# vankxr/qo-100-tools

Hardware: AMD Instinct MI355X
Metric: complex-IQ MSamples/s through 255-tap FIR (higher is better)
Workload: dtype f32

## Files before the change

include/if_fir_debug.h:

```cpp
#ifndef IF_FIR_DEBUG_H
#define IF_FIR_DEBUG_H

#include "if_fir.h"

#ifdef __cplusplus
extern "C" {
#endif

uint8_t if_fir_time_device(if_fir_ctx_t *pCtx, const void *pDevIn, void *pDevOut, uint64_t ullSamples,
                           uint32_t ulWarmup, uint32_t ulReps, float *pfMsPerCall);
uint32_t if_fir_debug_stamps(if_fir_ctx_t *pCtx, uint64_t *pullOut, uint32_t ulWords);
#define IF_FIR_DEBUG_TABLE_FLOATS 21632u
uint32_t if_fir_debug_fft_tables(const float *pfTaps, uint32_t ulTaps, uint32_t bComplexTaps, uint32_t ulDecimation,
                                 uint32_t ulNcoDelta, float *pfOut, uint32_t ulOutFloats);
uint32_t if_fir_debug_fft_tables_bank(const float *pfTaps, uint32_t ulTaps, uint32_t bComplexTaps, uint32_t ulBank, uint32_t ulParity,
                                      float *pfOut, uint32_t ulOutFloats);
uint32_t if_fir_debug_bank_tail(uint32_t ulDecimation, uint32_t bOwnCentres);
uint8_t if_fir_debug_bank_plan(const uint32_t *pulSlots, uint32_t ulChannels, uint32_t *pulOut);
#define IF_FIR_DEBUG_ODD_TABLE_FLOATS 10496u
uint32_t if_fir_debug_fft_tables_odd(const float *pfTaps, uint32_t ulTaps, uint32_t bComplexTaps, uint32_t ulDecimation,
                                     uint32_t ulNcoDelta, float *pfOut, uint32_t ulOutFloats);
uint8_t if_fir_debug_fft_schedule(uint64_t ullBlocks, uint32_t ulWorkgroups, uint32_t bSingleOk, int64_t *pllOut);
uint8_t if_fir_debug_queue_faults(if_fir_ctx_t *pCtx, uint32_t *pulFaults);
uint32_t if_fir_mc_debug_plan(uint32_t ulWorld, uint32_t ulChannels, uint32_t ulRank, uint64_t ullSamples,
                              uint32_t ulInBytes, uint32_t ulTaps, uint32_t ulDecimation, uint64_t ullConsumed,
                              uint64_t ullChunk, uint64_t *pullOut, uint32_t ulMaxOps);

uint8_t if_fir_debug_interp_config(if_fir_interp_t *pCtx, uint32_t bForceFull, uint32_t ulGridLimit);
uint8_t if_fir_debug_interp_seek(if_fir_interp_t *pCtx, uint64_t ullSamples);
uint32_t if_fir_debug_interp_tables(const float *pfTaps, uint32_t ulTaps, uint32_t bComplexTaps, float *pfOut, uint32_t ulOutFloats);
uint8_t if_fir_debug_interp_plan(uint32_t ulTaps, uint32_t ulInterpolation, uint32_t *pulRows, uint32_t *pulHistLen,
                                 uint32_t *pbFftOk);
uint8_t if_fir_debug_combiner_config(if_fir_combiner_t *pCtx, uint32_t ulGridLimit);
uint8_t if_fir_debug_combiner_seek(if_fir_combiner_t *pCtx, uint64_t ullSamples);
uint32_t if_fir_debug_combiner_tables(const float *pfTaps, uint32_t ulTaps, uint32_t bComplexTaps, double dCentre, uint32_t *pulGrid,
                                      int32_t *plResidual, float *pfOut, uint32_t ulOutFloats);
uint8_t if_fir_debug_resamp_config(if_fir_resamp_t *pCtx, uint32_t ulGridLimit, uint32_t *pulTileOutputs);
// ... 8 lines not shown
```

qo-100-tools_amd/csrc/if_fir_fft_dev.h:

```cpp
#pragma once
namespace if_fir
{

typedef float cf __attribute__((ext_vector_type(2)));
typedef float f2v __attribute__((ext_vector_type(2)));
typedef unsigned u2v __attribute__((ext_vector_type(2)));
typedef float f4v_t __attribute__((ext_vector_type(4)));

__device__ __forceinline__ cf cadd(cf a, cf b) { return a + b; }
__device__ __forceinline__ cf csub(cf a, cf b) { return a - b; }

template <bool CONJ>
__device__ __forceinline__ cf cmul_v(cf a, cf w)
{
    cf t, d;
    asm("v_pk_mul_f32 %0, %1, %2 op_sel_hi:[1,0]" : "=v"(t) : "v"(a), "v"(w));
    if (CONJ)
        asm("v_pk_fma_f32 %0, %1, %2, %3 op_sel:[1,1,0] op_sel_hi:[0,1,1] neg_hi:[0,1,0]" : "=v"(d) : "v"(a), "v"(w), "v"(t));
    else
        asm("v_pk_fma_f32 %0, %1, %2, %3 op_sel:[1,1,0] op_sel_hi:[0,1,1] neg_lo:[0,1,0]" : "=v"(d) : "v"(a), "v"(w), "v"(t));
    return d;
}
template <bool CONJ>
__device__ __forceinline__ cf cmul_s(cf a, cf w)
// ... 493 lines not shown
        const unsigned u = rem + off, qd = __umul24(u, magic) >> 18;
        const bool keep = (__umul24(qd, sub) == u) && in_range;
        return keep ? (qd - (rem ? 1u : 0u)) * 8u : 0xffffffffu;
    }
};

struct DevQueue
{
    char *qcur;
    char *qtail;
    char *qclaim;
    unsigned int *gqueue;
    unsigned int *tqueue;
    unsigned int *faultw;
    int lane;
    __device__ __forceinline__ unsigned long long *tailw() const { return reinterpret_cast<unsigned long long *>(qtail); }
    __device__ __forceinline__ unsigned tail_claim(unsigned simd)
    {
        unsigned c = 0;
        if (lane == 0)
            c = __hip_atomic_fetch_add(reinterpret_cast<unsigned int *>(qclaim) + simd, 1u, __ATOMIC_RELAXED, __HIP_MEMORY_SCOPE_WORKGROUP);
        return __builtin_amdgcn_readfirstlane(c);
    }
    __device__ __forceinline__ unsigned long long tail_add()
    {
        unsigned long long w = 0;
        if (lane == 0)
            w = __hip_atomic_fetch_add(tailw(), 1ull, __ATOMIC_RELAXED, __HIP_MEMORY_SCOPE_WORKGROUP);
        return uniform(w);
    }
// ... 48 lines not shown
    __device__ __forceinline__ unsigned ticket()
    {
        unsigned t = 0;
        if (lane == 0)
            t = atomicAdd(gqueue, 1u);
        return __builtin_amdgcn_readfirstlane(t);
    }
    __device__ __forceinline__ void fault()
    {
        if (lane == 0)
            atomicAdd(faultw, 1u);
    }
    __device__ __forceinline__ void pause() { __builtin_amdgcn_s_sleep(2); }
    __device__ __forceinline__ unsigned wgs() const { return gridDim.x; }
};
inline hipError_t fft_queue_select(const LaunchArgs &a, uint32_t *qsel)
{
    *qsel = 0;
    if (a.queue_base && a.queue_valid && *a.queue_valid)
        *qsel = *a.queue_base & 1u;
    else
    {
        const hipError_t e = hipMemsetAsync(a.queue, 0, 16, a.stream);
        if (e != hipSuccess)
            return e;
    }
    if (a.queue_base && a.queue_valid)
    {
        *a.queue_base = *qsel ^ 1u;
        *a.queue_valid = true;
    }
    return hipSuccess;
}
inline hipError_t fft_queue_launched(const LaunchArgs &a)
{
    const hipError_t le = hipGetLastError();
    if (le != hipSuccess && a.queue_valid)
        *a.queue_valid = false;
    return le;
}

template <bool PF = true>
__device__ __forceinline__ void inverse_tail256(cf (&a)[16], cf (&c)[16], const f2v *twe, const XAddr &xa, int lane)
{
    xst16<XROW>(xa.wx, a);
// ... 88 lines not shown
```

qo-100-tools_amd/csrc/if_fir_fft_kernel.inc:

```
template <int OVL_ROWS, bool DEC4, bool I16, bool NCO, int CHAN, bool DECN, bool ACC>
__global__ __launch_bounds__(512, 2) IF_FIR_LDS_SINGLE_READS void fir_fft_kernel(const f2v *__restrict__ in_, f2v *__restrict__ out,
                                                        const f2v *__restrict__ tables, const f2v *__restrict__ hist,
                                                        int HL, int64_t N, int32_t n0, int64_t M, int64_t nblocks,
                                                        int64_t nblocks_main, unsigned int *queue, unsigned long long *dbg, int32_t diag,
                                                        uint32_t nco_phi0, uint32_t nco_delta, chan_arg_t<CHAN> chan,
                                                        uint32_t qsel, void *__restrict__ hist_out,
                                                        int32_t decn, int32_t decn_n0, int64_t decn_m, int32_t in_shift)
{
    static_assert(!ACC || (tail_single(CHAN) && OVL_ROWS == 32), "accumulating store: single-channel pipelines, 32 overlap rows");
    static_assert(!DECN || (!DEC4 && CHAN == TAIL_FULL_OR_DEC4), "general decimation = the full-rate pipeline with a selecting store");
    static_assert(tail_valid(CHAN) && (CHAN == TAIL_FULL_OR_DEC4 || DEC4), "every named tail but the first is a decimating one");
    static_assert(tail_has_nco(CHAN) || !NCO, "channels at their own centres: no common offset on top; the decimate-by-4 bank takes no NCO either");
    static_assert(OVL_ROWS >= 4 || (!DEC4 && !ACC), "2 overlap rows: full-rate pipeline (D = 1, odd D) only");
    constexpr bool TAN = tail_wants_tan(CHAN, DEC4);
    constexpr bool TANF = !DEC4;
    constexpr int OVL = 64 * OVL_ROWS;
    constexpr int ISZ = I16 ? 4 : 8;
    const char *in = reinterpret_cast<const char *>(in_);
    constexpr int L = FFT_N - OVL;
    constexpr int LOUT = tail_lout(CHAN, DEC4, L);
    constexpr int EARLY_GROUPS = CHAN == TAIL_DEC4_SUB ? FFT_EARLY_GROUPS_SUB : FFT_EARLY_GROUPS;
    constexpr int LAUX = FFT_LOAD_AUX;
    constexpr int EDGE = OVL_ROWS;
    extern __shared__ __attribute__((aligned(16))) char smem[];
// ... 53 lines not shown
        }
        if (threadIdx.x < Q_RING)
            reinterpret_cast<unsigned long long *>(smem + LDS_Q + 16)[threadIdx.x] = queue_ring_init(threadIdx.x, blockIdx.x, gridDim.x);
        if (threadIdx.x < 4)
            reinterpret_cast<unsigned int *>(smem + LDS_QCLAIM)[threadIdx.x] = 0u;
        if (threadIdx.x == 0)
        {
            *reinterpret_cast<unsigned long long *>(smem + LDS_Q) = queue_cur_init(blockIdx.x, gridDim.x, true);
            *reinterpret_cast<unsigned long long *>(smem + LDS_QTAIL) = 0ull;
            if (blockIdx.x == 0)
            {
                queue[qsel ^ 1u] = 0u;
                queue[2u + (qsel ^ 1u)] = 0u;
            }
        }
    }
    __syncthreads();
    DevQueue dq{smem + LDS_Q, smem + LDS_QTAIL, smem + LDS_QCLAIM, queue + qsel, queue + 2 + qsel, queue + 4, lane};
    const unsigned simd = (unsigned)wid & 3u;
    if (wid == 0)
        queue_start(dq);
    if (hist_out && blockIdx.x == 0 && wid == 0)
    {
        const int64_t keep = (int64_t)HL;
        for (int64_t i = lane; i < keep; i += 64)
        {
            const int64_t gi = N - keep + i, hi = keep + gi;
            if constexpr (I16)
            {
                const int *src = reinterpret_cast<const int *>(in_), *hsrc = reinterpret_cast<const int *>(hist);
                reinterpret_cast<int *>(hist_out)[i] = gi >= 0 ? src[gi] : (hi >= 0 ? hsrc[hi] : 0);
            }
            else
// ... 41 lines not shown
        {                                                                                                        \
            dbg[(((blockIdx.x >> 6) * 2 + wid) * 32 + dbg_it) * 8 + (slot)] = __builtin_amdgcn_s_memrealtime();   \
            dbg[4096 + (((blockIdx.x >> 6) * 2 + wid) * 32 + dbg_it) * 8 + (slot)] = __builtin_amdgcn_s_memtime(); \
        }                                                                                                        \
    } while (0)
#else
#define FFT_STAMP(slot) (void)0
#endif
    unsigned long long st_r0 = 0, st_c0 = 0;
    if (dbg)
    {
        st_r0 = __builtin_amdgcn_s_memrealtime();
        st_c0 = __builtin_amdgcn_s_memtime();
    }
    const unsigned voff = (unsigned)lane * 8u;
    while (blk < nblocks)
    {
        FFT_STAMP(0);
        const int64_t s0 = rb(blk) * L - OVL + n0 - in_shift;
        if (!loaded && !(diag & 1))
        {
            if (s0 >= 0)
            {
                const srd_t srd = make_srd(in + s0 * ISZ, (N - s0) * ISZ);
#pragma unroll
                for (int rho = 0; rho < 4; rho++)
#pragma unroll
                    for (int j = 0; j < 16; j++)
                        load_row<I16, LAUX, EDGE>(r, srd, lane, 4 * j + rho);
            }
// ... 64 lines not shown
#pragma unroll
            for (int j = 0; j < 16; j++)
            {
                if (j == 0)
                    r[phys(i, j)] = t[j];
                else
                {
                    r[phys(i, j)] = cmul_v<false>(t[j], w2[j - 1]);
                }
            }
            }
        }
        FFT_STAMP(3);
        exchange2(r, xa);
        FFT_STAMP(4);
        const int64_t blk_next = queue_take(dq, simd, nblocks_main, nblocks);
        const int64_t s0n = rb(blk_next) * L - OVL + n0 - in_shift;
        const bool next_fast = (blk_next < nblocks) && (s0n >= 0) && !(diag & 1);
        const srd_t nsrd = make_srd(in + (next_fast ? s0n : 0) * ISZ, next_fast ? (N - s0n) * ISZ : 0);
        const int64_t obase = rb(blk) * LOUT;
        const srd_t osrd = make_srd(out + obase, (diag & 2) ? 0 : (M - obase) * 8);
        if constexpr (NCO && (CHAN == TAIL_BANK16_ALL || CHAN == TAIL_BANK8_ALL))
        {
            const float2 pb = phasor(nco_phi0 + nco_delta * (uint32_t)obase);
            if (lane == 0)
                *reinterpret_cast<cf *>(smem + LDS_QNCO + wid * 8) = (cf){pb.x, pb.y};
        }
        if constexpr (tail_is_bank(CHAN))
        {
#include "if_fir_fft_tails_bank.inc"
        }
// ... 22 lines not shown
```

qo-100-tools_amd/csrc/if_fir_fft_launch.inc:

```
template <int OVL_ROWS, bool DEC4, bool I16, bool NCO, int CHAN, bool DECN, bool ACC>
static constexpr auto fft_kernel_of()
{
#ifdef IF_FIR_FFT_DEC2_UNIT
    static_assert(tail_in_dec2_units(CHAN), "the decimate-by-2 units hold the decimate-by-2 tails only");
#else
    static_assert(!tail_in_dec2_units(CHAN), "the decimate-by-2 tails live in the decimate-by-2 units (launch_fft_dec2_rows)");
#endif
    return &fir_fft_kernel<OVL_ROWS, DEC4, I16, NCO, CHAN, DECN, ACC>;
}
template <int ROWS>
hipError_t launch_fft_dec2_rows(const LaunchArgs &a, int tail, bool nco, bool acc);
template <int OVL_ROWS, bool DEC4, bool I16, bool NCO, int CHAN, bool DECN, bool ACC>
static hipError_t launch_fft_t(const LaunchArgs &a)
{
    auto kern = fft_kernel_of<OVL_ROWS, DEC4, I16, NCO, CHAN, DECN, ACC>();
    constexpr int L = FFT_N - 64 * OVL_ROWS;
    constexpr int LOUT = tail_lout(CHAN, DEC4, L);
    static DeviceSetup setup;
    int ncus = 0;
    {
        const hipError_t e = device_setup(setup, a.device, reinterpret_cast<const void *>(kern), FFT_LDS_BYTES, &ncus);
        if (e != hipSuccess)
            return e;
    }
    constexpr int F = tail_factor(CHAN, DEC4);
    ChanArgs ca = a.chan ? *a.chan : ChanArgs{};
    ca.sub = tail_sub_word(CHAN, DEC4, a.D, ca.sub);
    const bool both = CHAN == TAIL_BANK8_ALL && (ca.sub & 2u);
    const int64_t m_rate = DECN ? a.N : CHAN == TAIL_BANK8_ALL ? a.M : (a.M - 1) * (int64_t)ca.sub + 1;
    const int32_t n0_rate = DECN ? 0 : a.n0;
    const int64_t nblocks = (a.M > 0 ? (m_rate + LOUT - 1) / LOUT : 0) * (both ? 2 : 1);
    if (nblocks <= 0)
        return hipSuccess;
    const int64_t wgs_max = (a.grid_limit > 0 && a.grid_limit < ncus) ? a.grid_limit : ncus;
    const FftLaunchPlan plan = fft_launch_plan(nblocks, wgs_max, !both && !(a.diag & 262144),
                                               (a.diag & 256) ? 0 : Q_TAIL_MAX_ROUNDS);
    uint32_t qsel = 0;
    {
        const hipError_t e = fft_queue_select(a, &qsel);
        if (e != hipSuccess)
            return e;
    }
    chan_arg_t<CHAN> cak;
    if constexpr (tail_is_bank(CHAN))
        cak = ca;
    else
        cak.sub = ca.sub;
    hipLaunchKernelGGL(kern, dim3((unsigned)plan.wgs), dim3(512), FFT_LDS_BYTES, a.stream,
                       reinterpret_cast<const f2v *>(a.in), reinterpret_cast<f2v *>(a.out),
                       reinterpret_cast<const f2v *>(a.fft_tables), reinterpret_cast<const f2v *>(a.hist_full), a.hist_len, a.N,
                       n0_rate, m_rate, nblocks, plan.nblocks_main, (unsigned int *)a.queue,
                       (unsigned long long *)a.dbg, (int32_t)a.diag | (plan.single ? 131072 : 0),
                       DECN ? 0u - a.nco_word * a.nco_abs0 : nco_phi0(a),
                       DECN ? 0u - a.nco_word : 0u - a.nco_word * (uint32_t)F,
                       cak, qsel, a.hist_out, (int32_t)a.D, (int32_t)a.n0, a.M,
                       (int32_t)a.in_shift);
    return fft_queue_launched(a);
}

enum { NCO_NEVER, NCO_BOTH, NCO_ALWAYS };
template <int ROWS, bool DEC4, int CHAN, bool DECN = false, bool ACC = false, int FORMS = tail_has_nco(CHAN) ? NCO_BOTH : NCO_NEVER>
static hipError_t launch_fft_form(const LaunchArgs &a, bool nco = false)
{
    static_assert(FORMS == NCO_NEVER || tail_has_nco(CHAN), "this tail has no NCO instantiation");
    if constexpr (FORMS == NCO_BOTH)
        switch ((a.in_i16 ? 2 : 0) | (nco ? 1 : 0))
        {
        case 0: return launch_fft_t<ROWS, DEC4, false, false, CHAN, DECN, ACC>(a);
        case 1: return launch_fft_t<ROWS, DEC4, false, true, CHAN, DECN, ACC>(a);
        case 2: return launch_fft_t<ROWS, DEC4, true, false, CHAN, DECN, ACC>(a);
        default: return launch_fft_t<ROWS, DEC4, true, true, CHAN, DECN, ACC>(a);
// ... 8 lines not shown
hipError_t launch_fft_dec2_rows(const LaunchArgs &a, int tail, bool nco, bool acc)
{
    const bool plain = tail == TAIL_DEC2;
    if constexpr (ROWS == 32)
        if (acc)
            return plain ? launch_fft_form<ROWS, true, TAIL_DEC2, false, true>(a, nco) : launch_fft_form<ROWS, true, TAIL_DEC2_SUB, false, true>(a, nco);
    if (acc)
        return hipErrorInvalidConfiguration;
    return plain ? launch_fft_form<ROWS, true, TAIL_DEC2>(a, nco) : launch_fft_form<ROWS, true, TAIL_DEC2_SUB>(a, nco);
}
#if defined(IF_FIR_FFT_ONLY)
__attribute__((used)) static auto *const if_fir_fft_only_kernel = &fir_fft_kernel<IF_FIR_FFT_ONLY>;
#elif defined(IF_FIR_FFT_HAZARD_PROBE)
template __global__ void fir_fft_kernel<IF_FIR_FFT_ROWS, true, false, false, TAIL_DEC2, false, false>(
    const f2v *, f2v *, const f2v *, const f2v *, int, int64_t, int32_t, int64_t, int64_t, int64_t, unsigned int *,
    unsigned long long *, int32_t, uint32_t, uint32_t, chan_arg_t<TAIL_DEC2>, uint32_t, void *, int32_t, int32_t, int64_t, int32_t);
#else
template hipError_t launch_fft_dec2_rows<IF_FIR_FFT_ROWS>(const LaunchArgs &a, int tail, bool nco, bool acc);
#endif
#else
template <int ROWS>
static hipError_t launch_fft_bank8(const LaunchArgs &a, const FftRoute &r)
{
    bool general = a.chan->general || r.sub != 1;
    for (uint32_t c = 0; c < a.chan->count; c++)
        general = general || (a.chan->bin[c] & 255u) || a.chan->pword[c] != (a.chan->bin[c] << 20) + a.nco_word;
    if (general)
        return launch_fft_form<ROWS, true, TAIL_BANK8_CHANNEL, false, false, NCO_ALWAYS>(a);
    const bool nco = a.nco_word != 0;
    const ChanArgs &cin = *a.chan;
    uint32_t pmask[2], rest = 0;
// ... 127 lines not shown
```

qo-100-tools_amd/csrc/if_fir_fft_queue.h:

```cpp
#pragma once
#include <stdint.h>

#if defined(__HIPCC__)
#define IF_FIR_Q_FN __host__ __device__ inline __attribute__((always_inline))
#else
#define IF_FIR_Q_FN inline __attribute__((always_inline))
#endif

namespace if_fir
{

constexpr unsigned QB = 8;
constexpr unsigned Q_AHEAD = 2;
constexpr unsigned Q_RING = 4;
constexpr unsigned Q_SPIN_LIMIT = 1u << 22;
constexpr int64_t Q_NONE = (int64_t)1 << 46;

IF_FIR_Q_FN unsigned long long queue_word(unsigned global_group, unsigned local_group, unsigned slot)
{
    return ((unsigned long long)global_group << 32) | ((unsigned long long)(local_group & 0xffffffu) << 8) | slot;
}
IF_FIR_Q_FN unsigned long long queue_entry(unsigned global_group, unsigned local_group)
{
    return ((unsigned long long)global_group << 32) | local_group;
// ... 93 lines not shown
                break;
            p.pause();
        }
    }
    p.fault();
    return Q_NONE;
}

constexpr int64_t Q_TAIL_MAX_ROUNDS = 6;
IF_FIR_Q_FN int64_t queue_main_blocks(int64_t nblocks, int64_t wgs, int64_t max_rounds = Q_TAIL_MAX_ROUNDS)
{
    const int64_t simds = 4 * wgs, p = nblocks / (2 * simds), rem = nblocks - 2 * p * simds;
    return (p >= 1 && p <= max_rounds && rem > 0 && rem <= simds) ? 2 * p * simds : nblocks;
}

struct FftLaunchPlan
{
    int64_t wgs;
    int64_t nblocks_main;
    int64_t tickets;
    bool single;
};
IF_FIR_Q_FN FftLaunchPlan fft_launch_plan(int64_t nblocks, int64_t wgs_max, bool single_ok, int64_t tail_rounds)
{
    const int64_t groups = (nblocks + QB - 1) / QB;
    FftLaunchPlan p;
    p.single = single_ok && nblocks <= (int64_t)QB * wgs_max;
    const int64_t want = p.single ? nblocks : groups;
    p.wgs = want < wgs_max ? want : wgs_max;
    if (p.wgs < 1)
        p.wgs = 1;
    p.nblocks_main = p.single ? nblocks : queue_main_blocks(nblocks, p.wgs, tail_rounds);
    p.tickets = groups + 2 * p.wgs;
    return p;
}

IF_FIR_Q_FN unsigned long long queue_cur_init(unsigned wg, unsigned wgs, bool static_first)
{
    return static_first ? queue_word(wgs + wg, 1, 0) : queue_word(wg, 0, 0);
}
IF_FIR_Q_FN unsigned long long queue_ring_init(unsigned i, unsigned wg, unsigned wgs)
{
    return i < Q_AHEAD ? queue_entry(i * wgs + wg, i) : ~0ull;
}

}
```

qo-100-tools_amd/csrc/if_fir_kernels.h:

```cpp
#pragma once
#include <hip/hip_runtime.h>
#include <stdint.h>

#include <mutex>

#include "if_fir_fft_route.h"

namespace if_fir
{

enum
{
    BACKEND_AUTO = 0,
    BACKEND_DIRECT = 1,
    BACKEND_TAPSPLIT = 2,
    BACKEND_GENERIC = 3,
    BACKEND_FFT = 4
};

constexpr int CHAN_MAX = 16;
struct ChanArgs
{
    uint32_t count;
    uint32_t slot[CHAN_MAX];
    float tw[CHAN_MAX][30];
    float rot0[CHAN_MAX][2];
    float2 *out[CHAN_MAX];
    uint32_t mask16;
    uint32_t rot_e;
    uint32_t sub;
    uint32_t bin[CHAN_MAX];
    uint32_t pword[CHAN_MAX];
    uint32_t abs0n0;
    uint32_t general;
};

struct LaunchArgs
{
    const void *in;
    void *out;
    const float *taps;
    const void *hist;
    const void *hist_full;
    int hist_len;
    int T, D;
    int in_i16;
    int ctaps;
    int64_t N;
    int32_t n0;
    int64_t M;
    int backend;
    int device;
    hipStream_t stream;
    const void *fft_tables;
    const void *fft_tables_b;
    int in_shift;
    void *queue;
    int diag;
    int grid_limit;
    void *dbg;
    uint32_t nco_word;
    uint32_t nco_abs0;
    void *hist_out;
    uint32_t *queue_base;
    bool *queue_valid;
    int no_fold;
    const ChanArgs *chan;
};

inline uint32_t nco_phi0(const LaunchArgs &a) { return 0u - a.nco_word * (a.nco_abs0 + (uint32_t)a.n0); }
inline uint32_t nco_delta(const LaunchArgs &a) { return 0u - a.nco_word * (uint32_t)a.D; }

#if defined(__HIPCC__)
__device__ __forceinline__ float2 nco_phasor(uint32_t ph)
{
    float sh, ch, sl, cl;
    sincospif((float)(ph >> 16) * (1.0f / 32768.0f), &sh, &ch);
    sincospif((float)(ph & 0xffffu) * (1.0f / 2147483648.0f), &sl, &cl);
    return make_float2(fmaf(ch, cl, -sh * sl), fmaf(sh, cl, ch * sl));
}
// ... 49 lines not shown
```

qo-100-tools_amd/csrc/if_fir_shim.cpp:

```cpp
#include <hip/hip_runtime.h>

#include <cmath>
#include <cstdarg>
#include <cstdio>
#include <cstdlib>
#include <cstring>
#include <new>

#include "if_fir.h"
#ifdef IF_FIR_DEVELOPMENT
#include "if_fir_debug.h"
#endif
#include "if_fir_kernels.h"
#ifdef IF_FIR_DEVELOPMENT
#include "if_fir_fft_queue.h"
#endif

#define IF_FIR_API extern "C" __attribute__((visibility("default")))

struct Tuning
{
    int schedule;
    uint32_t diag;
    int grid_limit;
    bool no_fold;
    bool inject_failure;
    bool needs_debug;
};
static Tuning decode_tuning(uint32_t v)
{
    Tuning t{};
    t.schedule = v <= 6 ? (int)v : 0;
    t.diag = (v >= 1000 && v < 2000) ? v - 1000 : (v >= 1000000 && v < 3000000) ? v - 1000000 : 0;
    t.grid_limit = (v > 2000 && v < 3000) ? (int)(v - 2000) : 0;
    t.no_fold = v == 3000;
    t.inject_failure = v == 4000;
    t.needs_debug = (v >= 1000 && v < 2000) || v == 4000 || v >= 1000000;
    return t;
}

struct if_fir_ctx
{
    int device;
    hipStream_t own_stream;
    hipStream_t stream;
    int T, D;
    int ctaps;
    int in_i16;
    uint32_t backend_req;
    uint32_t backend;
    Tuning tuning;
// ... 5 lines not shown
    uint64_t max_samples;
    void *d_stage_in;
    void *d_stage_out;
    hipStream_t copy_in, copy_out;
    hipEvent_t *chunk_ev;
    uint32_t chunk_ev_count;
    float tone[10];
    float *h_taps;
    uint32_t nco_word;
    float *h_eff;
    void *d_fft_tables;
    void *d_fft_tables_bank;
    void *d_queue;
    uint32_t queue_base;
    bool queue_valid;
    void *d_dbg;
    void *d_power;
    char info[128];
    mutable char err[256];
};

static thread_local char g_init_err[256] = "";

static void set_err(const if_fir_ctx *ctx, const char *fmt, ...)
{
    char *dst = ctx ? ctx->err : g_init_err;
    va_list ap;
    va_start(ap, fmt);
    vsnprintf(dst, 256, fmt, ap);
    va_end(ap);
}
// ... 190 lines not shown
            return 0;                                                                                \
        }                                                                                            \
    } while (0)

    INIT_TRY(hipSetDevice(lDevice));
    hipDeviceProp_t prop;
    INIT_TRY(hipGetDeviceProperties(&prop, lDevice));
    snprintf(ctx->info, sizeof(ctx->info), "%s %s cus=%d clock_mhz=%d lds_per_block=%zu", prop.name, prop.gcnArchName,
             prop.multiProcessorCount, prop.clockRate / 1000, (size_t)prop.sharedMemPerBlock);
    INIT_TRY(hipStreamCreateWithFlags(&ctx->own_stream, hipStreamNonBlocking));
    ctx->stream = ctx->own_stream;
    const size_t taps_padded = ((size_t)tap_floats + 63) / 64 * 64;
    INIT_TRY(hipMalloc((void **)&ctx->d_taps, sizeof(float) * taps_padded));
    INIT_TRY(hipMemset(ctx->d_taps, 0, sizeof(float) * taps_padded));
    INIT_TRY(hipMemcpy(ctx->d_taps, pfTaps, sizeof(float) * tap_floats, hipMemcpyHostToDevice));
    INIT_TRY(hipMalloc(&ctx->d_queue, 32));
    INIT_TRY(hipMemset(ctx->d_queue, 0, 32));
    ctx->hist_len = hist_len_for((int)ulTaps, (int)ulDecimation);
    const size_t hist_bytes = 8 * (size_t)(ctx->hist_len > 0 ? ctx->hist_len : 1);
    for (int i = 0; i < 2; i++)
    {
        INIT_TRY(hipMalloc(&ctx->d_hist[i], hist_bytes));
        INIT_TRY(hipMemset(ctx->d_hist[i], 0, hist_bytes));
    }
#undef INIT_TRY
    ctx->backend_req = IF_FIR_BACKEND_AUTO;
    ctx->backend = resolve_backend(ctx, IF_FIR_BACKEND_AUTO);
    if (ctx->backend == IF_FIR_BACKEND_HIP_FFT && !ensure_fft_tables(ctx))
    {
        snprintf(g_init_err, sizeof(g_init_err), "if_fir_init: %s", ctx->err);
        if_fir_destroy(ctx);
        return 0;
// ... 267 lines not shown
    a.n0 = (int32_t)n0;
    a.M = (int64_t)m;
    a.backend = (int)ctx->backend;
    a.device = ctx->device;
    a.stream = ctx->stream;
    a.fft_tables = ctx->d_fft_tables;
    a.fft_tables_b = (ctx->d_fft_tables && if_fir::fft_two_partitions(ctx->T))
                         ? static_cast<const float *>(ctx->d_fft_tables) + if_fir::FFT_TABLE_FLOATS : nullptr;
    a.queue = ctx->d_queue;
#ifdef IF_FIR_DEVELOPMENT
    a.dbg = ctx->d_dbg;
    const bool fft_var = ctx->backend == IF_FIR_BACKEND_HIP_FFT;
    a.diag = fft_var ? (int)ctx->tuning.diag : 0;
    a.grid_limit = fft_var ? ctx->tuning.grid_limit : 0;
    a.no_fold = ctx->tuning.no_fold;
#endif
    if (chan)
    {
        const bool slots16 = ctx->D == 16 && !chan->general;
        const uint32_t entries = slots16 ? 16u : chan->count;
        for (uint32_t c = 0; c < entries; c++)
        {
            const uint32_t slot = slots16 ? c : chan->slot[c];
            const uint32_t e = (uint32_t)((slot * ((ctx->consumed + n0) & 15u)) & 15u);
            chan->rot0[c][0] = (float)cos(-2.0 * M_PI * (double)e / 16.0);
            chan->rot0[c][1] = (float)sin(-2.0 * M_PI * (double)e / 16.0);
        }
        if (slots16)
        {
            chan->rot_e = (uint32_t)((ctx->consumed + n0) & 15u);
            chan->mask16 = 0;
            for (uint32_t c = 0; c < 16; c++)
                chan->mask16 |= chan->out[c] ? (1u << c) : 0u;
        }
        chan->abs0n0 = (uint32_t)(ctx->consumed + n0);
        a.chan = chan;
        const int kind = if_fir::fft_route_of(a).image.kind;
        if (kind == if_fir::FFT_IMAGE_BANK8 || kind == if_fir::FFT_IMAGE_BANK16)
            a.fft_tables = ctx->d_fft_tables_bank;
        if (kind == if_fir::FFT_IMAGE_BANK8)
            a.fft_tables_b = static_cast<const float *>(ctx->d_fft_tables_bank) + if_fir::FFT_TABLE_FLOATS;
    }
    a.queue_base = &ctx->queue_base;
    a.queue_valid = &ctx->queue_valid;
    const bool fused_history = ctx->backend == IF_FIR_BACKEND_HIP_FFT && m > 0 && ctx->hist_len > 0;
    a.hist_out = fused_history ? ctx->d_hist[ctx->hist_cur ^ 1] : nullptr;
    if (ctx->backend == IF_FIR_BACKEND_HIP_FFT)
        HIP_TRY(ctx, if_fir::launch_fft(a));
    else
        HIP_TRY(ctx, if_fir::launch_fir(a, ctx->tuning.schedule));
    if (!fused_history)
        HIP_TRY(ctx, if_fir::launch_history(in, ctx->d_hist[ctx->hist_cur], ctx->d_hist[ctx->hist_cur ^ 1], ctx->hist_len,
                                            (int64_t)n, ctx->in_i16, ctx->stream));
    if (commit)
    {
        ctx->hist_cur ^= 1;
        ctx->consumed += n;
    }
    return 1;
// ... 305 lines not shown
    HIP_TRY(pCtx, hipStreamSynchronize(pCtx->stream));
    HIP_TRY(pCtx, hipMemcpy(pulFaults, static_cast<const char *>(pCtx->d_queue) + 16, 4, hipMemcpyDeviceToHost));
    return 1;
}

IF_FIR_API uint8_t if_fir_debug_fft_schedule(uint64_t ullBlocks, uint32_t ulWorkgroups, uint32_t bSingleOk, int64_t *pllOut)
{
    if (!pllOut || !ullBlocks || !ulWorkgroups)
        return 0;
    const if_fir::FftLaunchPlan p =
        if_fir::fft_launch_plan((int64_t)ullBlocks, (int64_t)ulWorkgroups, bSingleOk != 0, if_fir::Q_TAIL_MAX_ROUNDS);
    pllOut[0] = p.wgs;
    pllOut[1] = p.nblocks_main;
    pllOut[2] = p.single ? 1 : 0;
    pllOut[3] = p.tickets;
    return 1;
}

#endif

IF_FIR_API uint8_t if_fir_power_device(if_fir_ctx_t *pCtx, const void *pDevIQ, uint64_t ullSamples, double *pdMeanPower)
{
    if (!pCtx || !pdMeanPower)
        return 0;
    *pdMeanPower = 0.0;
    if (ullSamples == 0)
        return 1;
    if (!pDevIQ || ((uintptr_t)pDevIQ & 15))
    {
        set_err(pCtx, "if_fir_power_device: the buffer must be a 16-byte aligned device pointer");
// ... 302 lines not shown
```

qo-100-tools_amd/if_fir.py:

```python
import ctypes
import os

import numpy as np

_HERE = os.path.dirname(os.path.abspath(__file__))
LIB_PATH = os.path.join(_HERE, "libif_fir.so")
DEV_LIB_PATH = os.path.join(_HERE, "libif_fir_dev.so")

INPUT_F32, INPUT_I16 = 0, 1
BACKEND_AUTO, BACKEND_HIP_DIRECT, BACKEND_HIP_TAPSPLIT, BACKEND_HIP_GENERIC, BACKEND_HIP_FFT = range(5)
WINDOW_RECT, WINDOW_HAMMING, WINDOW_HANN, WINDOW_BLACKMAN = range(4)

EXPORTS = [
    "if_bpf_design", "if_bpf_design_complex", "if_fir_init", "if_fir_init_complex", "if_fir_destroy", "if_fir_reset", "if_fir_set_backend", "if_fir_get_backend",
    "if_fir_set_tuning", "if_fir_set_input_format", "if_fir_set_stream", "if_fir_synchronize", "if_fir_last_error", "if_fir_out_count",
    "if_fir_process", "if_fir_process_device", "if_fir_synth_device", "if_fir_dev_alloc",
    "if_fir_dev_free", "if_fir_dev_upload", "if_fir_dev_download", "if_fir_device_info",
    "if_fir_set_nco", "if_fir_get_nco", "if_fir_channelizer_process_device", "if_fir_channelizer_process_device_freq", "if_fir_host_alloc", "if_fir_host_free",
    "if_fir_power_device",
    "if_fir_mc_owner", "if_fir_mc_unique_id", "if_fir_mc_init", "if_fir_mc_destroy", "if_fir_mc_reset",
    "if_fir_mc_set_input_format", "if_fir_mc_process_device", "if_fir_mc_channel_ctx", "if_fir_mc_last_error",
    "if_fir_mc_set_chunk_samples", "if_fir_mc_get_chunk_samples",
    "if_fir_interp_init", "if_fir_interp_init_complex", "if_fir_interp_destroy", "if_fir_interp_reset", "if_fir_interp_set_backend",
    "if_fir_interp_get_backend", "if_fir_interp_set_input_format", "if_fir_interp_set_nco", "if_fir_interp_get_nco",
# ... 2 lines not shown
    "if_fir_resamp_init", "if_fir_resamp_init_complex", "if_fir_resamp_destroy", "if_fir_resamp_reset", "if_fir_resamp_set_input_format",
    "if_fir_resamp_set_stream", "if_fir_resamp_synchronize", "if_fir_resamp_last_error", "if_fir_resamp_out_count",
    "if_fir_resamp_process", "if_fir_resamp_process_device",
    "if_fir_psd_init", "if_fir_psd_destroy", "if_fir_psd_reset", "if_fir_psd_set_input_format", "if_fir_psd_set_stream",
    "if_fir_psd_synchronize", "if_fir_psd_last_error", "if_fir_psd_frame_count", "if_fir_psd_process", "if_fir_psd_process_device",
    "if_fir_combiner_init", "if_fir_combiner_init_complex", "if_fir_combiner_destroy", "if_fir_combiner_reset", "if_fir_combiner_set_backend",
    "if_fir_combiner_get_backend", "if_fir_combiner_set_input_format", "if_fir_combiner_set_centres", "if_fir_combiner_get_centres",
    "if_fir_combiner_set_stream", "if_fir_combiner_synchronize", "if_fir_combiner_last_error", "if_fir_combiner_out_count",
    "if_fir_combiner_process", "if_fir_combiner_process_device",
    "if_fir_ddc_init", "if_fir_ddc_init_complex", "if_fir_ddc_destroy", "if_fir_ddc_reset", "if_fir_ddc_set_input_format",
    "if_fir_ddc_set_nco", "if_fir_ddc_get_nco", "if_fir_ddc_set_stream", "if_fir_ddc_synchronize", "if_fir_ddc_last_error",
    "if_fir_ddc_out_count", "if_fir_ddc_process", "if_fir_ddc_process_device",
]
DEV_EXPORTS = ["if_fir_time_device", "if_fir_debug_stamps", "if_fir_debug_fft_tables", "if_fir_debug_fft_tables_odd", "if_fir_debug_fft_tables_bank",
               "if_fir_debug_bank_plan", "if_fir_debug_bank_tail", "if_fir_debug_fft_schedule",
               "if_fir_mc_debug_plan", "if_fir_debug_queue_faults",
               "if_fir_debug_interp_config", "if_fir_debug_interp_seek", "if_fir_debug_interp_tables", "if_fir_debug_interp_plan",
               "if_fir_debug_resamp_config", "if_fir_debug_psd_plan",
               "if_fir_debug_combiner_config", "if_fir_debug_combiner_seek", "if_fir_debug_combiner_tables",
               "if_fir_debug_ddc_config"]
MC_ID_BYTES = 128


class PsdConfig(ctypes.Structure):
    _fields_ = [("ulSize", ctypes.c_uint32), ("ulHop", ctypes.c_uint32), ("ulSegments", ctypes.c_uint32), ("lFirstBin", ctypes.c_int32),
                ("ulBins", ctypes.c_uint32), ("fRefPower", ctypes.c_float), ("ulInputFormat", ctypes.c_uint32)]


class IfFirError(RuntimeError):
    pass
# ... 171 lines not shown
        L.if_fir_debug_interp_config.restype = u8
        L.if_fir_debug_interp_seek.argtypes = [vp, u64]
        L.if_fir_debug_interp_seek.restype = u8
        L.if_fir_debug_interp_tables.argtypes = [f32p, u32, u32, f32p, u32]
        L.if_fir_debug_interp_tables.restype = u32
        L.if_fir_debug_interp_plan.argtypes = [u32, u32, ctypes.POINTER(u32), ctypes.POINTER(u32), ctypes.POINTER(u32)]
        L.if_fir_debug_interp_plan.restype = u8
        L.if_fir_time_device.argtypes = [vp, vp, vp, u64, u32, u32, f32p]
        L.if_fir_time_device.restype = u8
        L.if_fir_debug_stamps.argtypes = [vp, ctypes.POINTER(u64), u32]
        L.if_fir_debug_stamps.restype = u32
        L.if_fir_debug_fft_tables.argtypes = [f32p, u32, u32, u32, u32, f32p, u32]
        L.if_fir_debug_fft_tables.restype = u32
        L.if_fir_debug_fft_schedule.argtypes = [u64, u32, u32, ctypes.POINTER(ctypes.c_int64)]
        L.if_fir_debug_fft_schedule.restype = u8
        L.if_fir_mc_debug_plan.argtypes = [u32, u32, u32, u64, u32, u32, u32, u64, u64, ctypes.POINTER(u64), u32]
        L.if_fir_mc_debug_plan.restype = u32
        L.if_fir_debug_queue_faults.argtypes = [vp, ctypes.POINTER(u32)]
        L.if_fir_debug_queue_faults.restype = u8
    _libs[path] = L
    return L


def _f32p(a):
    return a.ctypes.data_as(ctypes.POINTER(ctypes.c_float))


def _taps_arg(taps, complex_taps):
    taps = np.asarray(taps)
    if np.iscomplexobj(taps):
# ... 163 lines not shown
    def synth_device(self, dev_iq, first, samples, channel=0):
        self._check(self._L.if_fir_synth_device(self._ctx, ctypes.c_void_p(dev_iq), int(first), int(samples),
                                              int(channel)))

    def time_device(self, dev_in, dev_out, samples, warmup=3, reps=10):
        ms = ctypes.c_float(0)
        self._check(self._L.if_fir_time_device(self._ctx, ctypes.c_void_p(dev_in), ctypes.c_void_p(dev_out),
                                             int(samples), int(warmup), int(reps), ctypes.byref(ms)))
        return float(ms.value)

    def debug_queue_faults(self):
        n = ctypes.c_uint32(0)
        self._check(self._L.if_fir_debug_queue_faults(self._ctx, ctypes.byref(n)))
        return int(n.value)

    def debug_stamps(self, waves=None):
        if waves is None:
            self._L.if_fir_debug_stamps(self._ctx, None, 0)
            return None
        buf = np.zeros(4 * waves, dtype=np.uint64)
        n = self._L.if_fir_debug_stamps(self._ctx, buf.ctypes.data_as(ctypes.POINTER(ctypes.c_uint64)), buf.size)
        return buf[:n].reshape(-1, 4)

    def dev_alloc(self, nbytes):
        p = ctypes.c_void_p()
        self._check(self._L.if_fir_dev_alloc(self._ctx, ctypes.byref(p), int(nbytes)))
        return p.value

    def dev_free(self, ptr):
        self._check(self._L.if_fir_dev_free(self._ctx, ctypes.c_void_p(ptr)))
# ... 423 lines not shown
                                      ctypes.c_uint32(int(decimation)), ctypes.c_uint32(int(nco_delta) & 0xFFFFFFFF), _f32p(out),
                                      ctypes.c_uint32(out.size))
    if n != nfl:
        raise IfFirError("if_fir_debug_fft_tables_odd: (taps=%d, decimation=%d) is not served by the odd-decimation kernel" % (t, decimation))
    c = out.view(np.complex64)
    return {"g": c[0:3072], "tb": c[3072:3328], "tc": c[3328:4096], "twd": c[4096:5120], "twe": c[5120:5184], "ncob": c[5184:5248], "pht": c[5248:5504]}


def debug_fft_schedule(nblocks, workgroups=256, single_ok=True):
    out = (ctypes.c_int64 * 4)()
    if not dev_lib().if_fir_debug_fft_schedule(int(nblocks), int(workgroups), 1 if single_ok else 0, out):
        raise IfFirError("if_fir_debug_fft_schedule: bad arguments")
    return dict(zip(("wgs", "nblocks_main", "single", "tickets"), [int(v) for v in out]))


def mc_owner(channel, world):
    return int(lib().if_fir_mc_owner(int(channel), int(world)))


MC_CHUNK_UNIT = 215040
MC_NEVER_SPLIT = (1 << 64) - 1


def mc_debug_plan(world, channels, rank, samples, in_bytes=8, decimation=1, consumed=0, chunk=0, taps=255):
    n = dev_lib().if_fir_mc_debug_plan(int(world), int(channels), int(rank), int(samples), int(in_bytes), int(taps),
                                       int(decimation), int(consumed), int(chunk), None, 0)
    buf = np.zeros(8 * max(n, 1), dtype=np.uint64)
    dev_lib().if_fir_mc_debug_plan(int(world), int(channels), int(rank), int(samples), int(in_bytes), int(taps), int(decimation),
                                   int(consumed), int(chunk), buf.ctypes.data_as(ctypes.POINTER(ctypes.c_uint64)), n)
    keys = ("kind", "phase", "group", "peer", "channel", "chunk", "offset", "bytes")
# ... 81 lines not shown
```

Measured before the change: 597,200.

## Add per-block end phase to FFT work queue for finer tail balancing

For single-channel FFT pipelines, the last blocks of a launch are handed out one at a time through eight strided global atomic counters rather than in the usual grouped queue tickets. The goal is to shrink load imbalance at the end of the kernel, where workgroups finish grouped work at different times. It adds a larger queue buffer, an extra memset whenever the queue is invalid or dirty, and dirty-bit tracking, plus a per-block atomic on the end path. The phase is on by default (8 blocks per workgroup) once a launch has enough blocks.

```diff
diff --git a/include/if_fir_debug.h b/include/if_fir_debug.h
--- a/include/if_fir_debug.h
+++ b/include/if_fir_debug.h
@@ -21,6 +21,8 @@
 uint32_t if_fir_debug_fft_tables_odd(const float *pfTaps, uint32_t ulTaps, uint32_t bComplexTaps, uint32_t ulDecimation,
                                      uint32_t ulNcoDelta, float *pfOut, uint32_t ulOutFloats);
 uint8_t if_fir_debug_fft_schedule(uint64_t ullBlocks, uint32_t ulWorkgroups, uint32_t bSingleOk, int64_t *pllOut);
+uint8_t if_fir_debug_fft_end_phase(uint64_t ullBlocks, uint32_t ulWorkgroups, uint32_t bSingleOk, int32_t lEndPerWg, int64_t *pllOut);
+uint8_t if_fir_debug_fft_last_launch(const if_fir_ctx_t *pCtx, int64_t *pllOut);
 uint8_t if_fir_debug_queue_faults(if_fir_ctx_t *pCtx, uint32_t *pulFaults);
 uint32_t if_fir_mc_debug_plan(uint32_t ulWorld, uint32_t ulChannels, uint32_t ulRank, uint64_t ullSamples,
                               uint32_t ulInBytes, uint32_t ulTaps, uint32_t ulDecimation, uint64_t ullConsumed,
diff --git a/qo-100-tools_amd/csrc/if_fir_fft_dev.h b/qo-100-tools_amd/csrc/if_fir_fft_dev.h
--- a/qo-100-tools_amd/csrc/if_fir_fft_dev.h
+++ b/qo-100-tools_amd/csrc/if_fir_fft_dev.h
@@ -531,6 +531,14 @@
     unsigned int *tqueue;
     unsigned int *faultw;
     int lane;
+    unsigned int *equeue = nullptr;
+    __device__ __forceinline__ unsigned end_ticket(unsigned cls)
+    {
+        unsigned t = 0;
+        if (lane == 0)
+            t = atomicAdd(equeue + cls * Q_END_STRIDE, 1u);
+        return __builtin_amdgcn_readfirstlane(t);
+    }
     __device__ __forceinline__ unsigned long long *tailw() const { return reinterpret_cast<unsigned long long *>(qtail); }
     __device__ __forceinline__ unsigned tail_claim(unsigned simd)
     {
@@ -609,21 +617,35 @@
     __device__ __forceinline__ void pause() { __builtin_amdgcn_s_sleep(2); }
     __device__ __forceinline__ unsigned wgs() const { return gridDim.x; }
 };
-inline hipError_t fft_queue_select(const LaunchArgs &a, uint32_t *qsel)
+static_assert(FFT_QUEUE_BYTES == sizeof(unsigned int) * Q_WORDS, "LaunchArgs::queue holds the whole queue block");
+inline hipError_t fft_queue_select(const LaunchArgs &a, uint32_t *qsel, bool end_phase = false)
 {
     *qsel = 0;
-    if (a.queue_base && a.queue_valid && *a.queue_valid)
+    bool valid = a.queue_base && a.queue_valid && a.queue_end_dirty && *a.queue_valid;
+    if (valid && end_phase && ((*a.queue_end_dirty >> (*a.queue_base & 1u)) & 1u))
+        valid = false;
+    if (valid)
         *qsel = *a.queue_base & 1u;
     else
     {
-        const hipError_t e = hipMemsetAsync(a.queue, 0, 16, a.stream);
+        hipError_t e = hipMemsetAsync(a.queue, 0, 16, a.stream);
+        if (e == hipSuccess)
+            e = hipMemsetAsync(static_cast<unsigned int *>(a.queue) + Q_END_FIRST, 0, sizeof(unsigned int) * (Q_WORDS - Q_END_FIRST), a.stream);
         if (e != hipSuccess)
+        {
+            if (a.queue_valid)
+                *a.queue_valid = false;
             return e;
-    }
-    if (a.queue_base && a.queue_valid)
+        }
+        if (a.queue_end_dirty)
+            *a.queue_end_dirty = 0u;
+    }
+    if (a.queue_base && a.queue_valid && a.queue_end_dirty)
     {
         *a.queue_base = *qsel ^ 1u;
         *a.queue_valid = true;
+        if (end_phase)
+            *a.queue_end_dirty = (*a.queue_end_dirty | (1u << *qsel)) & ~(1u << (*qsel ^ 1u));
     }
     return hipSuccess;
 }
diff --git a/qo-100-tools_amd/csrc/if_fir_fft_kernel.inc b/qo-100-tools_amd/csrc/if_fir_fft_kernel.inc
--- a/qo-100-tools_amd/csrc/if_fir_fft_kernel.inc
+++ b/qo-100-tools_amd/csrc/if_fir_fft_kernel.inc
@@ -5,8 +5,9 @@
                                                         int64_t nblocks_main, unsigned int *queue, unsigned long long *dbg, int32_t diag,
                                                         uint32_t nco_phi0, uint32_t nco_delta, chan_arg_t<CHAN> chan,
                                                         uint32_t qsel, void *__restrict__ hist_out,
-                                                        int32_t decn, int32_t decn_n0, int64_t decn_m, int32_t in_shift)
+                                                        int32_t decn, int32_t decn_n0, int64_t decn_m, int32_t in_shift, uint32_t qend)
 {
+    constexpr bool END = tail_single(CHAN);
     static_assert(!ACC || (tail_single(CHAN) && OVL_ROWS == 32), "accumulating store: single-channel pipelines, 32 overlap rows");
     static_assert(!DECN || (!DEC4 && CHAN == TAIL_FULL_OR_DEC4), "general decimation = the full-rate pipeline with a selecting store");
     static_assert(tail_valid(CHAN) && (CHAN == TAIL_FULL_OR_DEC4 || DEC4), "every named tail but the first is a decimating one");
@@ -91,9 +92,13 @@
                 queue[2u + (qsel ^ 1u)] = 0u;
             }
         }
+        if constexpr (END)
+            if (qend != 0u && blockIdx.x == 0 && threadIdx.x < Q_END_CLASSES)
+                queue[Q_END_FIRST + ((qsel ^ 1u) * Q_END_CLASSES + threadIdx.x) * Q_END_STRIDE] = 0u;
     }
     __syncthreads();
-    DevQueue dq{smem + LDS_Q, smem + LDS_QTAIL, smem + LDS_QCLAIM, queue + qsel, queue + 2 + qsel, queue + 4, lane};
+    DevQueue dq{smem + LDS_Q, smem + LDS_QTAIL, smem + LDS_QCLAIM, queue + qsel, queue + 2 + qsel, queue + 4, lane,
+                queue + Q_END_FIRST + qsel * (Q_END_CLASSES * Q_END_STRIDE)};
     const unsigned simd = (unsigned)wid & 3u;
     if (wid == 0)
         queue_start(dq);
@@ -165,6 +170,7 @@
         st_c0 = __builtin_amdgcn_s_memtime();
     }
     const unsigned voff = (unsigned)lane * 8u;
+    bool groups_done = false;
     while (blk < nblocks)
     {
         FFT_STAMP(0);
@@ -259,7 +265,7 @@
         FFT_STAMP(3);
         exchange2(r, xa);
         FFT_STAMP(4);
-        const int64_t blk_next = queue_take(dq, simd, nblocks_main, nblocks);
+        const int64_t blk_next = queue_next<END>(dq, simd, blockIdx.x, nblocks_main, nblocks, qend, groups_done);
         const int64_t s0n = rb(blk_next) * L - OVL + n0 - in_shift;
         const bool next_fast = (blk_next < nblocks) && (s0n >= 0) && !(diag & 1);
         const srd_t nsrd = make_srd(in + (next_fast ? s0n : 0) * ISZ, next_fast ? (N - s0n) * ISZ : 0);
diff --git a/qo-100-tools_amd/csrc/if_fir_fft_launch.inc b/qo-100-tools_amd/csrc/if_fir_fft_launch.inc
--- a/qo-100-tools_amd/csrc/if_fir_fft_launch.inc
+++ b/qo-100-tools_amd/csrc/if_fir_fft_launch.inc
@@ -33,11 +33,19 @@
     if (nblocks <= 0)
         return hipSuccess;
     const int64_t wgs_max = (a.grid_limit > 0 && a.grid_limit < ncus) ? a.grid_limit : ncus;
-    const FftLaunchPlan plan = fft_launch_plan(nblocks, wgs_max, !both && !(a.diag & 262144),
-                                               (a.diag & 256) ? 0 : Q_TAIL_MAX_ROUNDS);
+    int64_t end_blocks = 0;
+    const FftLaunchPlan plan = fft_launch_plan_end(nblocks, wgs_max, !both && !(a.diag & 262144), (a.diag & 256) ? 0 : Q_TAIL_MAX_ROUNDS,
+                                                   tail_single(CHAN), a.end_per_wg, &end_blocks);
+    if (a.plan_out)
+    {
+        a.plan_out[0] = nblocks;
+        a.plan_out[1] = plan.wgs;
+        a.plan_out[2] = plan.nblocks_main - end_blocks;
+        a.plan_out[3] = end_blocks;
+    }
     uint32_t qsel = 0;
     {
-        const hipError_t e = fft_queue_select(a, &qsel);
+        const hipError_t e = fft_queue_select(a, &qsel, end_blocks > 0);
         if (e != hipSuccess)
             return e;
     }
@@ -49,12 +57,12 @@
     hipLaunchKernelGGL(kern, dim3((unsigned)plan.wgs), dim3(512), FFT_LDS_BYTES, a.stream,
                        reinterpret_cast<const f2v *>(a.in), reinterpret_cast<f2v *>(a.out),
                        reinterpret_cast<const f2v *>(a.fft_tables), reinterpret_cast<const f2v *>(a.hist_full), a.hist_len, a.N,
-                       n0_rate, m_rate, nblocks, plan.nblocks_main, (unsigned int *)a.queue,
+                       n0_rate, m_rate, nblocks, plan.nblocks_main - end_blocks, (unsigned int *)a.queue,
                        (unsigned long long *)a.dbg, (int32_t)a.diag | (plan.single ? 131072 : 0),
                        DECN ? 0u - a.nco_word * a.nco_abs0 : nco_phi0(a),
                        DECN ? 0u - a.nco_word : 0u - a.nco_word * (uint32_t)F,
                        cak, qsel, a.hist_out, (int32_t)a.D, (int32_t)a.n0, a.M,
-                       (int32_t)a.in_shift);
+                       (int32_t)a.in_shift, (uint32_t)end_blocks);
     return fft_queue_launched(a);
 }
 
@@ -93,7 +101,7 @@
 #elif defined(IF_FIR_FFT_HAZARD_PROBE)
 template __global__ void fir_fft_kernel<IF_FIR_FFT_ROWS, true, false, false, TAIL_DEC2, false, false>(
     const f2v *, f2v *, const f2v *, const f2v *, int, int64_t, int32_t, int64_t, int64_t, int64_t, unsigned int *,
-    unsigned long long *, int32_t, uint32_t, uint32_t, chan_arg_t<TAIL_DEC2>, uint32_t, void *, int32_t, int32_t, int64_t, int32_t);
+    unsigned long long *, int32_t, uint32_t, uint32_t, chan_arg_t<TAIL_DEC2>, uint32_t, void *, int32_t, int32_t, int64_t, int32_t, uint32_t);
 #else
 template hipError_t launch_fft_dec2_rows<IF_FIR_FFT_ROWS>(const LaunchArgs &a, int tail, bool nco, bool acc);
 #endif
diff --git a/qo-100-tools_amd/csrc/if_fir_fft_queue.h b/qo-100-tools_amd/csrc/if_fir_fft_queue.h
--- a/qo-100-tools_amd/csrc/if_fir_fft_queue.h
+++ b/qo-100-tools_amd/csrc/if_fir_fft_queue.h
@@ -131,6 +131,42 @@
     return (p >= 1 && p <= max_rounds && rem > 0 && rem <= simds) ? 2 * p * simds : nblocks;
 }
 
+constexpr unsigned Q_END_CLASSES = 8;
+constexpr unsigned Q_END_STRIDE = 32;
+constexpr unsigned Q_END_FIRST = 32;
+constexpr unsigned Q_WORDS = Q_END_FIRST + 2 * Q_END_CLASSES * Q_END_STRIDE;
+constexpr int64_t Q_END_PER_WG = 8;
+
+IF_FIR_Q_FN unsigned queue_end_classes(unsigned wgs) { return wgs < Q_END_CLASSES ? wgs : Q_END_CLASSES; }
+template <class P>
+IF_FIR_Q_FN int64_t queue_end_take(P &p, unsigned wg, int64_t end_first, int64_t nblocks)
+{
+    const unsigned classes = queue_end_classes(p.wgs()), cls = wg & (Q_END_CLASSES - 1u);
+    const unsigned t = p.end_ticket(cls);
+    const int64_t blk = end_first + (int64_t)classes * t + cls;
+    return blk < nblocks ? blk : Q_NONE;
+}
+
+template <bool END, class P>
+IF_FIR_Q_FN int64_t queue_next(P &p, unsigned simd, unsigned wg, int64_t nblocks_main, int64_t nblocks, unsigned qend, bool &groups_done)
+{
+    if constexpr (END)
+    {
+        if (qend != 0u)
+        {
+            if (!groups_done)
+            {
+                const int64_t blk = queue_take(p, simd, nblocks_main, nblocks_main);
+                if (blk < nblocks_main)
+                    return blk;
+                groups_done = true;
+            }
+            return queue_end_take(p, wg, nblocks_main, nblocks);
+        }
+    }
+    return queue_take(p, simd, nblocks_main, nblocks);
+}
+
 struct FftLaunchPlan
 {
     int64_t wgs;
@@ -152,6 +188,24 @@
     return p;
 }
 
+IF_FIR_Q_FN int64_t queue_end_blocks(int64_t nblocks, const FftLaunchPlan &plan, int64_t per_wg, bool force)
+{
+    if (plan.single || plan.nblocks_main != nblocks || per_wg <= 0)
+        return 0;
+    if (!force && nblocks < 2 * 4 * plan.wgs * (Q_TAIL_MAX_ROUNDS + 1))
+        return 0;
+    const int64_t room = nblocks - (int64_t)QB * plan.wgs, want = per_wg * plan.wgs;
+    return room <= 0 ? 0 : want < room ? want : room;
+}
+IF_FIR_Q_FN FftLaunchPlan fft_launch_plan_end(int64_t nblocks, int64_t wgs_max, bool single_ok, int64_t tail_rounds, bool end_ok,
+                                              int end_per_wg, int64_t *end_blocks)
+{
+    const bool force = end_ok && end_per_wg > 256;
+    const FftLaunchPlan p = fft_launch_plan(nblocks, wgs_max, single_ok, force ? 0 : tail_rounds);
+    *end_blocks = (!end_ok || end_per_wg < 0) ? 0 : queue_end_blocks(nblocks, p, end_per_wg > 0 ? (end_per_wg & 255) : Q_END_PER_WG, force);
+    return p;
+}
+
 IF_FIR_Q_FN unsigned long long queue_cur_init(unsigned wg, unsigned wgs, bool static_first)
 {
     return static_first ? queue_word(wgs + wg, 1, 0) : queue_word(wg, 0, 0);
diff --git a/qo-100-tools_amd/csrc/if_fir_kernels.h b/qo-100-tools_amd/csrc/if_fir_kernels.h
--- a/qo-100-tools_amd/csrc/if_fir_kernels.h
+++ b/qo-100-tools_amd/csrc/if_fir_kernels.h
@@ -35,6 +35,8 @@
     uint32_t general;
 };
 
+constexpr size_t FFT_QUEUE_BYTES = 128 + 2 * 8 * 128;
+
 struct LaunchArgs
 {
     const void *in;
@@ -64,6 +66,9 @@
     void *hist_out;
     uint32_t *queue_base;
     bool *queue_valid;
+    uint32_t *queue_end_dirty;
+    int end_per_wg;
+    int64_t *plan_out;
     int no_fold;
     const ChanArgs *chan;
 };
diff --git a/qo-100-tools_amd/csrc/if_fir_shim.cpp b/qo-100-tools_amd/csrc/if_fir_shim.cpp
--- a/qo-100-tools_amd/csrc/if_fir_shim.cpp
+++ b/qo-100-tools_amd/csrc/if_fir_shim.cpp
@@ -25,8 +25,14 @@
     int grid_limit;
     bool no_fold;
     bool inject_failure;
+    int end_per_wg;
     bool needs_debug;
 };
+static bool end_variant(uint32_t v)
+{
+    const uint32_t k = v - 5000u;
+    return v > 5000 && v < 5512 && ((k & 255u) == 4 || (k & 255u) == 8 || (k & 255u) == 16);
+}
 static Tuning decode_tuning(uint32_t v)
 {
     Tuning t{};
@@ -35,6 +41,7 @@
     t.grid_limit = (v > 2000 && v < 3000) ? (int)(v - 2000) : 0;
     t.no_fold = v == 3000;
     t.inject_failure = v == 4000;
+    t.end_per_wg = v == 5000 ? -1 : end_variant(v) ? (int)(v - 5000) : 0;
     t.needs_debug = (v >= 1000 && v < 2000) || v == 4000 || v >= 1000000;
     return t;
 }
@@ -70,7 +77,9 @@
     void *d_queue;
     uint32_t queue_base;
     bool queue_valid;
+    uint32_t queue_end_dirty;
     void *d_dbg;
+    int64_t last_plan[4];
     void *d_power;
     char info[128];
     mutable char err[256];
@@ -291,8 +300,8 @@
     INIT_TRY(hipMalloc((void **)&ctx->d_taps, sizeof(float) * taps_padded));
     INIT_TRY(hipMemset(ctx->d_taps, 0, sizeof(float) * taps_padded));
     INIT_TRY(hipMemcpy(ctx->d_taps, pfTaps, sizeof(float) * tap_floats, hipMemcpyHostToDevice));
-    INIT_TRY(hipMalloc(&ctx->d_queue, 32));
-    INIT_TRY(hipMemset(ctx->d_queue, 0, 32));
+    INIT_TRY(hipMalloc(&ctx->d_queue, if_fir::FFT_QUEUE_BYTES));
+    INIT_TRY(hipMemset(ctx->d_queue, 0, if_fir::FFT_QUEUE_BYTES));
     ctx->hist_len = hist_len_for((int)ulTaps, (int)ulDecimation);
     const size_t hist_bytes = 8 * (size_t)(ctx->hist_len > 0 ? ctx->hist_len : 1);
     for (int i = 0; i < 2; i++)
@@ -590,6 +599,9 @@
     a.diag = fft_var ? (int)ctx->tuning.diag : 0;
     a.grid_limit = fft_var ? ctx->tuning.grid_limit : 0;
     a.no_fold = ctx->tuning.no_fold;
+    a.end_per_wg = fft_var ? ctx->tuning.end_per_wg : 0;
+    memset(ctx->last_plan, 0, sizeof(ctx->last_plan));
+    a.plan_out = ctx->last_plan;
 #endif
     if (chan)
     {
@@ -619,6 +631,7 @@
     }
     a.queue_base = &ctx->queue_base;
     a.queue_valid = &ctx->queue_valid;
+    a.queue_end_dirty = &ctx->queue_end_dirty;
     const bool fused_history = ctx->backend == IF_FIR_BACKEND_HIP_FFT && m > 0 && ctx->hist_len > 0;
     a.hist_out = fused_history ? ctx->d_hist[ctx->hist_cur ^ 1] : nullptr;
     if (ctx->backend == IF_FIR_BACKEND_HIP_FFT)
@@ -954,6 +967,27 @@
     pllOut[1] = p.nblocks_main;
     pllOut[2] = p.single ? 1 : 0;
     pllOut[3] = p.tickets;
+    return 1;
+}
+
+
+IF_FIR_API uint8_t if_fir_debug_fft_end_phase(uint64_t ullBlocks, uint32_t ulWorkgroups, uint32_t bSingleOk, int32_t lEndPerWg, int64_t *pllOut)
+{
+    if (!pllOut || !ullBlocks || !ulWorkgroups)
+        return 0;
+    int64_t e = 0;
+    const if_fir::FftLaunchPlan p = if_fir::fft_launch_plan_end((int64_t)ullBlocks, (int64_t)ulWorkgroups, bSingleOk != 0,
+                                                                if_fir::Q_TAIL_MAX_ROUNDS, true, (int)lEndPerWg, &e);
+    pllOut[0] = p.nblocks_main - e;
+    pllOut[1] = e;
+    return 1;
+}
+
+IF_FIR_API uint8_t if_fir_debug_fft_last_launch(const if_fir_ctx_t *pCtx, int64_t *pllOut)
+{
+    if (!pCtx || !pllOut)
+        return 0;
+    memcpy(pllOut, pCtx->last_plan, sizeof(pCtx->last_plan));
     return 1;
 }
 
diff --git a/qo-100-tools_amd/if_fir.py b/qo-100-tools_amd/if_fir.py
--- a/qo-100-tools_amd/if_fir.py
+++ b/qo-100-tools_amd/if_fir.py
@@ -40,6 +40,7 @@
 ]
 DEV_EXPORTS = ["if_fir_time_device", "if_fir_debug_stamps", "if_fir_debug_fft_tables", "if_fir_debug_fft_tables_odd", "if_fir_debug_fft_tables_bank",
                "if_fir_debug_bank_plan", "if_fir_debug_bank_tail", "if_fir_debug_fft_schedule",
+               "if_fir_debug_fft_end_phase", "if_fir_debug_fft_last_launch",
                "if_fir_mc_debug_plan", "if_fir_debug_queue_faults",
                "if_fir_debug_interp_config", "if_fir_debug_interp_seek", "if_fir_debug_interp_tables", "if_fir_debug_interp_plan",
                "if_fir_debug_resamp_config", "if_fir_debug_psd_plan",
@@ -241,6 +242,11 @@
         L.if_fir_debug_fft_tables.restype = u32
         L.if_fir_debug_fft_schedule.argtypes = [u64, u32, u32, ctypes.POINTER(ctypes.c_int64)]
         L.if_fir_debug_fft_schedule.restype = u8
+        if hasattr(L, "if_fir_debug_fft_end_phase"):
+            L.if_fir_debug_fft_end_phase.argtypes = [u64, u32, u32, ctypes.c_int32, ctypes.POINTER(ctypes.c_int64)]
+            L.if_fir_debug_fft_end_phase.restype = u8
+            L.if_fir_debug_fft_last_launch.argtypes = [vp, ctypes.POINTER(ctypes.c_int64)]
+            L.if_fir_debug_fft_last_launch.restype = u8
         L.if_fir_mc_debug_plan.argtypes = [u32, u32, u32, u64, u32, u32, u32, u64, u64, ctypes.POINTER(u64), u32]
         L.if_fir_mc_debug_plan.restype = u32
         L.if_fir_debug_queue_faults.argtypes = [vp, ctypes.POINTER(u32)]
@@ -434,6 +440,11 @@
         self._check(self._L.if_fir_debug_queue_faults(self._ctx, ctypes.byref(n)))
         return int(n.value)
 
+    def debug_fft_last_launch(self):
+        out = (ctypes.c_int64 * 4)()
+        self._check(self._L.if_fir_debug_fft_last_launch(self._ctx, out))
+        return dict(zip(("blocks", "wgs", "groups", "end"), [int(v) for v in out]))
+
     def debug_stamps(self, waves=None):
         if waves is None:
             self._L.if_fir_debug_stamps(self._ctx, None, 0)
@@ -887,6 +898,13 @@
     return dict(zip(("wgs", "nblocks_main", "single", "tickets"), [int(v) for v in out]))
 
 
+def debug_fft_end_phase(nblocks, workgroups=256, single_ok=True, end_per_wg=0):
+    out = (ctypes.c_int64 * 2)()
+    if not dev_lib().if_fir_debug_fft_end_phase(int(nblocks), int(workgroups), 1 if single_ok else 0, int(end_per_wg), out):
+        raise IfFirError("if_fir_debug_fft_end_phase: bad arguments")
+    return int(out[0]), int(out[1])
+
+
 def mc_owner(channel, world):
     return int(lib().if_fir_mc_owner(int(channel), int(world)))
 
```

Result: no change. 601,600 (median of 6 runs) (+0.7%).
